# TobiaMarcucci/warm-start-hybrid-mpc

Measured on AMD Instinct MI355X. Metric: QP subproblems/sec, cart-pole-with-walls N=20 synthetic frontier, higher is better.
Workload: dtype f64

## Files before the change

### warm-start-hybrid-mpc_amd/csrc/hmpc_capi.hip

```cpp
#include <hip/hip_runtime.h>

#include <cmath>
#include <cstdio>
#include <cstdlib>
#include <cstring>
#include <memory>
#include <string>
#include <utility>
#include <vector>

#include "hmpc_device.h"

#include "hmpc_kernel.hip"
#include "hmpc_jit.h"
#include "hmpc_host.h"
#include "hmpc_shift.hip"
#include "hmpc_certify.hip"
#include "hmpc_branch.hip"
#include "hmpc_search.hip"

#define HMPC_CHECK_NODES 64

namespace {

struct StageHost {
    int m, mg;
    std::vector<double> C, h, scale;
    std::vector<int> rptr, rcol, cptr, crow, gptr, grow;
    std::vector<double> rval, cval, gval;
// ... 78 lines not shown
             "p.ring=%d;p.nd=%d;p.ndp=%d;p.ns=%d;p.nd_magic=%uu;p.nn_magic=%uu;p.split_lds=%d;p.static_rows=%d;p.polish_l1=%d;",
             p.nx, p.nu, p.nub, p.nuc, p.nz, p.T, p.nc, p.ncL, p.nT, p.mreg, p.Toff, p.M, p.Mpad, p.n, p.ne, p.nq, p.nr, p.nqT, p.n_primal, p.n_dual,
             p.mreg_magic, p.nnz0, p.nng0, p.reg.m, p.reg.mg, p.kcol, p.ngram, p.ring, p.nd, p.ndp, p.ns, p.nd_magic, p.nn_magic, p.split_lds,
             p.static_rows, p.polish_l1);
    return b;
}

static bool hmpc_sized_enabled()
{
    if (getenv("HMPC_FORCE_GENERIC") || getenv("HMPC_FORCE_BIG")) return false;
    if (const char *e = getenv("HMPC_JIT")) { if (atoi(e) == 0) return false; }
    if (const char *e = getenv("HMPC_JIT_SIZED")) { if (atoi(e) == 0) return false; }
    return true;
}

bool hmpc_jit_prepare_sized(const DevProb &p, hmpc_cfg (&cfg)[3], std::vector<void *> &libs, int &count_out, std::vector<std::string> *built)
{
    const std::string fields = hmpc_sized_fields(p);
    hmpc_jit_shape shapes[3];
    int slot[3], count = 0;
    int only = -1;
    if (const char *e = getenv("HMPC_WAVES")) { const int nw = atoi(e); only = nw == 1 || nw == 2 || nw == 4 ? hmpc_cfg_index(nw) : -1; }
    for (int c = 0; c < 3; c++) {
        const hmpc_kernel_choice &k = cfg[c].k;
        if (k.kc > 0) {
            int kf = 0, kb = 0, kt = 0;
            if (!hmpc_static_slots(p, k.waves, kf, kb, kt)) continue;
            if (kt < 1) kt = 1;
            shapes[count] = hmpc_jit_shape{p.nx, p.nu, p.nub, kf, kb, kt, k.waves, k.kc, fields};
            slot[count++] = c;
            continue;
        }
        if (k.big && c != (only >= 0 ? only : 2)) continue;
        int rs = p.Mpad / (WAVE << c), rs_max = 16;
        if (const char *e = getenv("HMPC_JIT_SIZED_ROWS")) rs_max = atoi(e);
        if (rs > rs_max) rs = 0;
        shapes[count] = hmpc_jit_shape{k.big ? -1 : 0, -1, 0, rs, 0, 0, 1 << c, 0, fields};
        slot[count++] = c;
    }
    if (!getenv("HMPC_JIT_SCHED")) {
        const uint64_t hsh = hmpc_jit::source_hash();
        for (int i = 0; i < count; i++) {
            hmpc_jit_shape probe = shapes[i];
            probe.ilp = 1;
// ... 53 lines not shown
{
    static const bool once = [] {
        if (getenv("HMPC_BACKTRACE")) { signal(SIGSEGV, hmpc_fatal_signal); signal(SIGABRT, hmpc_fatal_signal); signal(SIGBUS, hmpc_fatal_signal); }
        return true;
    }();
    (void)once;
}

namespace {

struct HostProblem {
    DevProb p{};
    StageHost reg;
    std::vector<double> ccv, Ct, ht, sct, P, PT, Cdn, sval;
    std::vector<int> cci, ei, ej, drow, rinfo, sptr, srow, nrow;
};

void split_rows(HostProblem &hp)
{
    DevProb &p = hp.p;
    const int nz = p.nz;
    const std::vector<double> &C = hp.reg.C;
    std::vector<int> &drow = hp.drow, &rinfo = hp.rinfo, &sptr = hp.sptr, &srow = hp.srow, &nrow = hp.nrow;
    std::vector<double> &sval = hp.sval, &Cdn = hp.Cdn;
    rinfo.assign(p.mreg, 0);
    sptr.assign(nz + 1, 0);
    sval.assign(p.mreg, 0.0);
    for (int r = 0; r < p.mreg; r++) {
        int cnt = 0, col = 0;
        for (int j = 0; j < nz; j++)
// ... 48 lines not shown
    p.dbg = getenv("HMPC_DBG") ? atoi(getenv("HMPC_DBG")) : 0;
    p.polish = opt ? opt->polish : 1;
    p.ptol = opt && opt->polish_tol > 0 ? opt->polish_tol : 1e-4;

    build_stage(q, q.F, q.G, q.h, q.nc, reg);
    p.reg.m = reg.m;
    p.reg.mg = reg.mg;
    p.mreg_magic = (unsigned)((0x100000000ULL + p.mreg - 1) / p.mreg);
    p.nnz0 = (int)reg.rcol.size();
    hp.ccv.assign((size_t)nz * HMPC_KC_STRIDE, 0.0);
    hp.cci.assign((size_t)nz * HMPC_KC_STRIDE, 0);
    p.kcol = 0;
    for (int j = 0; j < nz; j++) {
        const int len = reg.cptr[j + 1] - reg.cptr[j];
        if (len > p.kcol) p.kcol = len;
        for (int k = 0; k < len && k < HMPC_KC_STRIDE; k++) {
            hp.ccv[(size_t)j * HMPC_KC_STRIDE + k] = reg.cval[reg.cptr[j] + k];
            hp.cci[(size_t)j * HMPC_KC_STRIDE + k] = reg.crow[reg.cptr[j] + k];
        }
    }
    p.static_rows = (p.kcol <= HMPC_KC_STRIDE && p.mreg <= 255) ? 1 : 0;
    for (int r = 0; r < q.nc; r++) {
        int cnt = 0;
        for (int j = 0; j < nu; j++) cnt += reg.C[(size_t)r * nz + nx + j] != 0.0;
        if (cnt > 2) p.static_rows = 0;
    }
    p.nng0 = (int)reg.grow.size();
    for (int r = 0; r < q.nc; r++) {
        bool same = q.h_Tm1[r] == q.h[r];
        for (int j = 0; j < nx && same; j++) same = q.F_Tm1[r * nx + j] == q.F[r * nx + j];
// ... 38 lines not shown
        }
    p.cs = big > 0 ? 1.0 / big : 1.0;
    for (auto &v : P) v *= p.cs;
    for (auto &v : PT) v *= p.cs;
    {
        double cmin = 1.0;
        for (int i = 0; i < nz; i++) if (P[(size_t)i * nz + i] > 0) cmin = std::fmin(cmin, P[(size_t)i * nz + i]);
        for (int i = 0; i < nx; i++) if (PT[(size_t)i * nx + i] > 0) cmin = std::fmin(cmin, PT[(size_t)i * nx + i]);
        p.polish_l1 = cmin >= 1e-2 ? 1 : 0;
    }

    {
        std::vector<int> ei, ej;
        for (int i = 0; i < nz; i++)
            for (int j = 0; j <= i; j++) { ei.push_back(i); ej.push_back(j); }
        std::vector<int> order;
        for (int pass = 0; pass < 2; pass++)
            for (int e = 0; e < p.ne; e++)
                if ((reg.gptr[e + 1] > reg.gptr[e]) == (pass == 0)) order.push_back(e);
        p.ngram = 0;
        for (int e = 0; e < p.ne; e++) p.ngram += reg.gptr[e + 1] > reg.gptr[e];
        std::vector<int> gptr2(1, 0), grow2;
        std::vector<double> gval2;
        for (int e : order) {
            hp.ei.push_back(ei[e]); hp.ej.push_back(ej[e]);
            for (int k = reg.gptr[e]; k < reg.gptr[e + 1]; k++) { grow2.push_back(reg.grow[k]); gval2.push_back(reg.gval[k]); }
            gptr2.push_back((int)grow2.size());
        }
        reg.gptr.swap(gptr2); reg.grow.swap(grow2); reg.gval.swap(gval2);
        if (p.ngram > 128) p.static_rows = 0;
    }
    split_rows(hp);
    if (p.M >= 65536 || p.mreg >= 65536) return fail(HMPC_ETOOBIG, "more than 65535 constraint rows per node");
    return HMPC_OK;
}

int choose_kernels(DevProb &p, int lds_max, hmpc_cfg (&cfg)[3], std::vector<void *> &libs, int &jit_kernels, std::vector<std::string> *built)
{
    p.split_lds = 0;
    p.ring = 1;
    if (p.nz >= 16) {
        const bool big = hmpc_lds_bytes(p, 0, 0) > LDS_PER_CU || getenv("HMPC_FORCE_BIG");
        p.split_lds = 1;
        if (hmpc_lds_bytes(p, 0, big ? 1 : 0) > LDS_PER_CU) p.split_lds = 0;
    }
    for (int r = 2; r >= 1; r--) {
        p.ring = r;
        if (hmpc_lds_bytes(p, 0, 1) <= LDS_PER_CU) break;
    }
    if (const char *e = getenv("HMPC_RING")) {
        const int r = atoi(e);
        if (r >= 1 && r <= 2) p.ring = r;
// ... 3 lines not shown
        const bool sized = pass == 0 && hmpc_sized_enabled();
        if (pass == 0 && !sized) continue;
        for (int c = 0; c < 3; c++) { jit[c] = hmpc_kernel_choice{}; cfg[c] = hmpc_cfg{}; }
        jit_kernels = 0;
        if (sized) hmpc_jit_register_shapes(p, jit, LDS_PER_CU);
        for (int c = 0; c < 3; c++) {
            hmpc_cfg &cf = cfg[c];
            cf.k = hmpc_pick_kernel(p, 1 << c, jit);
            cf.lds = hmpc_lds_bytes(p, cf.k.kc, cf.k.big);
            if (cf.lds > LDS_PER_CU || (lds_max > 0 && cf.lds > (size_t)lds_max)) {
                char msg[256];
                snprintf(msg, sizeof msg, "problem needs %zu bytes of LDS per node, more than one CU has (%d)", cf.lds, lds_max > 0 ? lds_max : (int)LDS_PER_CU);
                return fail(HMPC_ETOOBIG, msg);
            }
        }
        if (!sized || hmpc_jit_prepare_sized(p, cfg, libs, jit_kernels, built)) break;
    }
    return HMPC_OK;
}

int resident_grid(size_t lds, int cus, const char *per_cu_env)
{
    int per_cu = (int)(LDS_PER_CU / lds);
    if (per_cu > 8) per_cu = 8;
    if (per_cu_env && atoi(per_cu_env) > 0) per_cu = atoi(per_cu_env);
    return (cus > 0 ? cus : 256) * per_cu;
}

struct CheckLayout {
    size_t obj, dobj, status, iters, idx, primal, dual, x0, fix, mirror, total;
};
// ... 129 lines not shown
    hmpc_install_backtrace();
    g_err.clear();
    if (!q || !out) return fail(HMPC_EINVAL, "null problem or output pointer");
    HostProblem hp;
    int rc = build_host_problem(*q, opt, hp);
    if (rc) return rc;
    int dev = opt ? opt->device : -1;
    if (dev < 0 && hipGetDevice(&dev) != hipSuccess) return fail(HMPC_EDEVICE, "no HIP device available");
    if (hipSetDevice(dev) != hipSuccess) return fail(HMPC_EDEVICE, "hipSetDevice failed");
    std::unique_ptr<hmpc_handle> h(new hmpc_handle());
    h->device = dev;
    h->dp = hp.p;
    int cus = 0, lds_max = 0;
    (void)hipDeviceGetAttribute(&cus, hipDeviceAttributeMultiprocessorCount, dev);
    (void)hipDeviceGetAttribute(&lds_max, hipDeviceAttributeMaxSharedMemoryPerBlock, dev);
    if ((rc = choose_kernels(h->dp, lds_max, h->cfg, h->jit_libs, h->jit_kernels, nullptr))) return rc;
    if ((rc = setup_device(h.get(), hp, *q, cus, lds_max))) return rc;
    if ((rc = hmpc_certify_setup(h.get(), cus))) return rc;
    *out = h.release();
    return HMPC_OK;
}

extern "C" int hmpc_jit_build_problem(const hmpc_problem *q, const hmpc_options *opt, char *paths, int32_t paths_len)
{
    g_err.clear();
    if (!q) return fail(HMPC_EINVAL, "null problem or output pointer");
    HostProblem hp;
    int rc = build_host_problem(*q, opt, hp);
    if (rc) return rc;
    hmpc_cfg cfg[3];
    std::vector<void *> libs;
    std::vector<std::string> built;
    int jit_kernels = 0;
    if ((rc = choose_kernels(hp.p, 0, cfg, libs, jit_kernels, &built))) return rc;
    if (paths && paths_len > 0) {
        std::string all;
        for (const std::string &b : built) all += b + "\n";
        snprintf(paths, (size_t)paths_len, "%s", all.c_str());
    }
    return HMPC_OK;
}

extern "C" int hmpc_destroy(hmpc_handle *h)
{
    if (!h) return HMPC_OK;
    (void)hipSetDevice(h->device);
    (void)hipDeviceSynchronize();
    delete h;
    return HMPC_OK;
// ... 355 lines not shown
```

### warm-start-hybrid-mpc_amd/csrc/hmpc_jit.h

```cpp
#ifndef HMPC_JIT_H
#define HMPC_JIT_H

#include <dlfcn.h>
#include <spawn.h>
#include <sys/stat.h>
#include <sys/wait.h>
#include <unistd.h>

#include <atomic>
#include <cerrno>
#include <climits>
#include <cstdint>
#include <cstdio>
#include <cstdlib>
#include <cstring>
#include <fstream>
#include <sstream>
#include <string>
#include <vector>

extern char **environ;

struct hmpc_jit_shape {
    int nx, nu, nub, kf, kb, kt, nw, kc;
    std::string sized;
    int ilp = 0;
};

namespace hmpc_jit {

inline std::string dir_of_library()
{
    Dl_info info;
    static int anchor;
    if (!dladdr((void *)&anchor, &info) || !info.dli_fname) return ".";
    std::string p = info.dli_fname;
    const size_t s = p.rfind('/');
    return s == std::string::npos ? "." : p.substr(0, s);
}

inline bool exists(const std::string &p) { struct stat st; return stat(p.c_str(), &st) == 0; }
// ... 103 lines not shown

inline uint64_t fnv(const std::string &t)
{
    uint64_t hsh = 1469598103934665603ull;
    for (char ch : t) { hsh ^= (unsigned char)ch; hsh *= 1099511628211ull; }
    return hsh;
}

inline std::string name_of(const hmpc_jit_shape &s, uint64_t hsh0)
{
    char b[160];
    const std::string fl = sched_flags(s) + "|" + safe_flags();
    const uint64_t hsh = hsh0 ^ fnv(fl);
    if (!s.sized.empty() && s.nx > 0) {
        snprintf(b, sizeof b, "hmpc_s_reg_%d_%d_%d_%d_%d_%d_w%d_kc%d%s_%016llx_%016llx", s.nx, s.nu, s.nub, s.kf, s.kb, s.kt, s.nw, s.kc, "",
                 (unsigned long long)fnv(s.sized), (unsigned long long)hsh);
        return b;
    }
    if (!s.sized.empty()) {
        snprintf(b, sizeof b, "hmpc_s_%s_w%d_r%d_%016llx_%016llx", s.nx < 0 ? "stream" : "generic", s.nw, s.kf, (unsigned long long)fnv(s.sized), (unsigned long long)hsh);
        return b;
    }
    return std::string();
}

inline std::vector<std::string> scrubbed_environment()
{
    static const char *const drop[] = {"LD_PRELOAD=", "ROCP", "ROCPROFILER", "ROCTRACER", "ROCTX", "HSA_TOOLS_LIB=", "HSA_TOOLS_REPORT_LOAD_FAILURE=", "HIP_TOOLS_LIB="};
    std::vector<std::string> env;
    for (char **e = environ; e && *e; e++) {
        bool keep = true;
// ... 24 lines not shown
    return tag;
}
inline unsigned next_build_seq() { static std::atomic<unsigned> n{0}; return n.fetch_add(1); }

inline pid_t start_build(const hmpc_jit_shape &s, const std::string &cache, uint64_t hsh, std::string &err, unsigned seq)
{
    const std::string base = cache + "/" + name_of(s, hsh), so = base + ".so";
    if (exists(so)) return 0;
    if (!exists(source_dir() + "/hmpc_kernel.hip")) { err = "kernel sources not found in " + source_dir(); return -1; }
    if (access(compiler().c_str(), X_OK) != 0) { err = "no compiler at " + compiler(); return -1; }
    const std::string tag = build_tag(seq);
    const std::string src = base + tag + ".hip", tmp = base + tag + ".tmp.so";
    {
        std::ofstream out(src);
        out << "// generated by hmpc_jit.h\n#define HMPC_KERNEL_ONLY\n#define hmpc_qp_kernel hmpc_qp_kernel_jit\n";
        if (s.nx > 0) out << "#define HMPC_JIT_KC " << s.kc << "\n";
        if (!s.sized.empty()) out << "#define HMPC_SIZED(p) " << s.sized << "\n";
        std::stringstream args;
        if (s.nx > 0) args << s.nx << ", " << s.nu << ", " << s.nub << ", " << s.kf << ", " << s.kb << ", " << s.kt << ", " << s.nw;
        else args << s.nx << ", -1, 0, " << s.kf << ", 0, 0, " << s.nw;
        out << "#include \"hmpc_device.h\"\n#include \"hmpc_kernel.hip\"\nHMPC_INSTANCE(" << args.str() << ")\nextern \"C\" void hmpc_jit_kernels(void **cold, void **warm)\n{\n    *cold = (void *)hmpc_qp_kernel<"
            << args.str() << ", false>;\n    *warm = (void *)hmpc_qp_kernel<" << args.str() << ", true>;\n}\nextern \"C\" const char *hmpc_jit_sized(void) { return \"" << s.sized << "\"; }\n";
        if (!out) { err = "cannot write " + src; return -1; }
    }
    const std::string cmd = compiler() + " --offload-arch=" + arch() + " -O3 -fPIC -std=c++17 -ffp-contract=fast -Wno-pass-failed " + quoted_flags(s) + " -I '" + include_dir() + "' -I '" +
                            source_dir() + "' -shared -Wl,-Bsymbolic -o '" + tmp + "' '" + src + "' > '" + base + tag + ".log' 2>&1 && mv '" + tmp + "' '" + so + "'";
    pid_t pid = -1;
    const char *argv[] = {"sh", "-c", cmd.c_str(), nullptr};
    const std::vector<std::string> env = scrubbed_environment();
    std::vector<char *> envp;
    for (const std::string &e : env) envp.push_back(const_cast<char *>(e.c_str()));
// ... 62 lines not shown
```

### warm-start-hybrid-mpc_amd/csrc/hmpc_kernel.hip

```cpp
#include <hip/hip_runtime.h>
#include <math.h>
#include <stdint.h>
#include <type_traits>

#include "hmpc_device.h"

#define WAVE 64
#define HMPC_REFINE_FROM_IT 12
#define HMPC_POLISH_RHO 1e5
#define HMPC_POLISH_RHO2 1e7
#define HMPC_POLISH_DELTA 1e-10
#define HMPC_RHO_OF(level) ((level) == 1 ? HMPC_POLISH_RHO2 : HMPC_POLISH_RHO)
#define HMPC_POLISH_ITERS 5
#define HMPC_POLISH_ROUNDS 6
#define HMPC_POLISH_ROUNDS_LAST 10
#define HMPC_ESC_MAX 2
#define HMPC_ESC_ITERS 6
#define HMPC_ESC_ENABLED(D) true
#define HMPC_LAM0_ROW 1
#ifndef HMPC_STABLE_DEN
#define HMPC_STABLE_DEN 1
#endif
#ifndef HMPC_PAIR
#define HMPC_PAIR 1
// ... 322 lines not shown
                a1 += c1 * v1;
                a2 += c2 * v2;
                a3 += c3 * v3;
            }
            for (; j < nz; j++) a0 += c[j] * v[j];
            return (a0 + a1) + (a2 + a3);
        }
    }
    if (lr < p.mreg) return row_dot(stage_lists<D>(S), lr, v);
    const int nz = D::nz(p);
    const double *c = p.Ct + (size_t)(lr - p.mreg) * nz;
    double a = 0;
    for (int j = 0; j < nz; j++) a += c[j] * v[j];
    return a;
}
template <class D> DEV double ccol_dot(const DevProb &p, const Lds &S, int t, int j, const ldsd *base)
{
    double a;
    if constexpr (D::kKC > 0) {
        const ldsd *eb = base + t * p.mreg, *cv = S.ccv + j * D::kKC;
        const ldsb *ci = S.cci + j * D::kKC;
        constexpr int H = D::kKC / 2;
        static_assert(D::kKC % 2 == 0, "padded columns come in two halves");
        double a0 = 0, a1 = 0;
#pragma unroll
        for (int hb = 0; hb < D::kKC; hb += H) {
            int idx[H];
            double cc[H], ee[H];
#pragma unroll
            for (int q = 0; q < H; q++) idx[q] = ci[hb + q];
#pragma unroll
            for (int q = 0; q < H; q++) cc[q] = cv[hb + q];
            HMPC_FENCE();
#pragma unroll
            for (int q = 0; q < H; q++) { HMPC_CHK(idx[q] >= 0 && idx[q] < p.mreg && j >= 0 && j < D::nz(p) && t >= 0 && t < p.T, 1); ee[q] = eb[idx[q]]; }
            HMPC_FENCE();
#pragma unroll
            for (int q = 0; q < H; q++) {
                if (q & 1) a1 += cc[q] * ee[q];
                else a0 += cc[q] * ee[q];
            }
        }
        a = a0 + a1;
    } else if (D::kBig && S.Cdn) {
        const int nz = D::nz(p);
        const ldsd *eb = base + t * p.mreg, *c = S.Cdn + j;
        double a0 = 0, a1 = 0;
        int r = 0;
        for (; r + 2 <= p.nd; r += 2) {
            a0 += c[r * nz] * eb[S.drow[r]];
            a1 += c[(r + 1) * nz] * eb[S.drow[r + 1]];
        }
        if (r < p.nd) a0 += c[r * nz] * eb[S.drow[r]];
// ... 807 lines not shown
{
    constexpr int NX = D::kNX, NU = D::kNU, NUB = D::kNUB, NUC = NU - NUB, NZ = NX + NU, NE = NZ * (NZ + 1) / 2;
    static_assert(NZ <= 16, "the register recursions broadcast inside one row of 16 lanes");
    constexpr int NXS = NX * (NX + 1) / 2, LMS = LM_STAGE(NX, NU), KG = D::kKC, GH = KG / 2;
    const int T = p.T;
    FSTAMP_DECL;
    LANE_OPAQUE(lane);
    if (lane == 0) S.flag[0] = 0;
    if (D::kNW == 1 || lane < WAVE) {
        const int ng = p.ngram;
        const bool has = lane < ng;
        const int ge = has ? lane : 0;
        const int gi = S.ei[ge], gj = S.ej[ge];
        const int gp0 = S.L0.gptr[ge], glen = has ? S.L0.gptr[ge + 1] - gp0 : 0;
        const double pij = S.P[gi * NZ + gj];
        ldsd *TG = S.Mm + NZ * NZ;
        for (int q = ng + lane; q < NE; q += WAVE) {
            const int i = S.ei[q], j = S.ej[q];
            const double a = S.P[i * NZ + j];
            S.Mm[i * NZ + j] = a;
            S.Mm[j * NZ + i] = a;
        }
        if (S.term_on) {
            const ldsd *Dt = S.e + p.Toff;
            if (p.nT == 0) {
                for (int q = lane; q < NZ * NZ; q += WAVE) TG[q] = 0.0;
            }
            for (int r0 = 0; r0 < p.nT; r0 += WAVE) {
                const int row = r0 + lane;
                const bool ok = row < p.nT;
// ... 23 lines not shown
#pragma unroll
        for (int i = 0; i < NX; i++) pn[i] = lane < NX ? S.PT[i * NX + lane] : 0.0;
        if (lane < NX) {
#pragma unroll
            for (int i = 0; i < NX; i++)
                if (i >= lane) S.Pr[T * NXS + sym(i, lane)] = pn[i];
        }
        int bad = 0;
        for (int t = T - 1; t >= 0; t--) {
            const ldsi *fx = S.fix + t * NUB;
            ldsd *Lm = S.Lm + t * LMS;
            int fxv[NUB];
#pragma unroll
            for (int b = 0; b < NUB; b++) fxv[b] = fx[b];
            double g0 = pij, g1 = 0.0;
            {
                const ldsd *Dt = S.e + t * p.mreg;
#pragma unroll
                for (int hb = 0; hb < KG; hb += GH) {
                    int idx[GH];
                    double gv[GH], dv[GH];
#pragma unroll
                    for (int q = 0; q < GH; q++) {
                        const int qq = gp0 + (hb + q < glen ? hb + q : 0);
                        idx[q] = S.L0.grow[qq];
                        gv[q] = S.L0.gval[qq];
                    }
                    HMPC_FENCE();
#pragma unroll
                    for (int q = 0; q < GH; q++) { HMPC_CHK(idx[q] >= 0 && idx[q] < p.mreg, 2); dv[q] = Dt[idx[q]]; }
                    HMPC_FENCE();
#pragma unroll
                    for (int q = 0; q < GH; q++) {
                        const double term = hb + q < glen ? gv[q] * dv[q] : 0.0;
                        if (q & 1) g1 += term;
                        else g0 += term;
                    }
                }
            }
            if (has) {
                S.Mm[gi * NZ + gj] = g0 + g1;
                S.Mm[gj * NZ + gi] = g0 + g1;
            }
            if (ng > WAVE) {
                const bool has2 = WAVE + lane < ng;
                const int ge2 = has2 ? WAVE + lane : 0;
                const int gi2 = S.ei[ge2], gj2 = S.ej[ge2];
                const int gq0 = S.L0.gptr[ge2], glen2 = has2 ? S.L0.gptr[ge2 + 1] - gq0 : 0;
                const ldsd *Dt = S.e + t * p.mreg;
                double h0 = S.P[gi2 * NZ + gj2], h1 = 0.0;
#pragma unroll
                for (int q = 0; q < KG; q++) {
                    const int qq = gq0 + (q < glen2 ? q : 0);
                    const double term = q < glen2 ? S.L0.gval[qq] * Dt[S.L0.grow[qq]] : 0.0;
// ... 650 lines not shown
    }
    __syncthreads();
    FSTAMP(10);
}

template <class D, int RS, class RM>
DEV void kkt_solve_reg(const DevProb &p, const Lds &S, Rows<RS> &R, const RM &rm, int lane, const ldsd *gsrc, double gs, bool usex0,
                       const ldsd *csrc, double cs, bool useb, ldsd *dw, ldsd *dlam, ldsd *dnuf FSTAMP_ARGS)
{
    constexpr int NX = D::kNX, NU = D::kNU, NUB = D::kNUB, NUC = NU - NUB, NZ = NX + NU;
    constexpr int NXS = NX * (NX + 1) / 2, LMS = LM_STAGE(NX, NU);
    const int T = p.T;
    FSTAMP_DECL;
    LANE_OPAQUE(lane);
    term_cols<D, RM>(p, S, lane, S.e);
    for (int o = lane; o < T * NZ; o += D::kNT) {
        const int t = o / NZ, j = o - t * NZ;
        const double a = (gsrc ? gs * gsrc[o] : 0.0) + ccol_dot<D>(p, S, t, j, S.e);
        S.g[o] = (useb ? S.g[o] : 0.0) - a;
    }
    for (int o = lane; o < T * NX; o += D::kNT) {
        const int t = o / NX, i = o - t * NX;
        double a = 0.0;
        if (csrc) {
#pragma unroll
            for (int l = 0; l < NX; l++) a += S.Pr[(t + 1) * NXS + sym(i, l)] * (cs * csrc[t * NX + l]);
        }
        S.pv[o] = a;
    }
    double pvr = 0.0;
    if (lane < NX) {
        pvr = -(gsrc ? gs * gsrc[T * NZ + lane] : 0.0);
        S.pv[T * NX + lane] = pvr;
    }
    __syncthreads();
// ... 150 lines not shown
                }
            }
        }
    }
    __syncthreads();
    const bool own_g = gsrc && gsrc != S.g;
    term_cols<D, RM>(p, S, lane, S.e);
    for (int o = lane; o < T * NUB; o += D::kNT) {
        const int t = o / NUB, b = o - t * NUB;
        double a = 0;
        if (S.fix[o] >= 0) {
            const int c = NX + NUC + b;
            a = own_g ? gs * gsrc[t * NZ + c] : 0.0;
#pragma unroll
            for (int j = 0; j < NZ; j++) a -= S.P[c * NZ + j] * dw[t * NZ + j];
            a -= ccol_dot<D>(p, S, t, c, S.e);
#pragma unroll
            for (int l = 0; l < NX; l++) a += S.AB[l * NZ + c] * dlam[(t + 1) * NX + l];
        }
        dnuf[o] = a;
    }
    if constexpr (HMPC_LAM0_ROW) {
        if (lane < NX) {
            double a = own_g ? gs * gsrc[lane] : 0.0;
#pragma unroll
            for (int j = 0; j < NZ; j++) a -= S.P[lane * NZ + j] * dw[j];
            a -= ccol_dot<D>(p, S, 0, lane, S.e);
#pragma unroll
            for (int l = 0; l < NX; l++) a += S.AB[l * NZ + lane] * dlam[NX + l];
            dlam[lane] = a;
        }
    }
    __syncthreads();
    FSTAMP(10);
}

template <class D, int RS, class RM>
DEV double kkt_solve_reg_pair(const DevProb &p, const Lds &S, Rows<RS> &R, const RM &rm, int lane, double tau FSTAMP_ARGS)
{
    constexpr int NX = D::kNX, NU = D::kNU, NUB = D::kNUB, NUC = NU - NUB, NZ = NX + NU;
    constexpr int NXS = NX * (NX + 1) / 2, LMS = LM_STAGE(NX, NU);
    const int T = p.T;
    const int nslot = RS;
    ldsd *pv2 = S.edyn;
    FSTAMP_DECL;
    LANE_OPAQUE(lane);
    ROWS_BEGIN(k, rw)
        S.e[rw.e] = R.D(k, rw.e) * rm.h(p, S, k, rw);
    ROWS_END
    __syncthreads();
    term_cols<D, RM>(p, S, lane, S.e);
    for (int o = lane; o < T * NZ; o += D::kNT) {
        const int t = o / NZ, j = o - t * NZ;
        S.g[o] = S.g[o] - ccol_dot<D>(p, S, t, j, S.e);
    }
    for (int o = lane; o < (T + 1) * NX; o += D::kNT) S.pv[o] = 0.0;
    __syncthreads();
    ROWS_BEGIN(k, rw)
        double v = 0;
        const double d = R.D(k, rw.e);
        if (d != 0.0) {
            const double sr = R.s(k, rw.e), zr = d * sr;
            const double rc = sr - rm.h(p, S, k, rw) * tau + rm.dot(p, S, k, rw, S.w);
            const double dsr = sr * zr;
            v = dsr * frcp(sr) - 1.0 * (d * rc);
        }
        S.e[rw.e] = v;
        R.dz(k, rw.e) = v;
    ROWS_END
    __syncthreads();
    term_cols<D, RM>(p, S, lane, S.e);
    for (int o = lane; o < T * NZ; o += D::kNT) {
        const int t = o / NZ, j = o - t * NZ;
        const double a = -1.0 * S.rd[o] + ccol_dot<D>(p, S, t, j, S.e);
        S.w2[o] = 0.0 - a;
    }
    for (int o = lane; o < T * NX; o += D::kNT) {
        const int t = o / NX, i = o - t * NX;
        double a = 0.0;
#pragma unroll
        for (int l = 0; l < NX; l++) a += S.Pr[(t + 1) * NXS + sym(i, l)] * (-1.0 * S.rdyn[t * NX + l]);
        pv2[o] = a;
    }
    double pvrA = 0.0, pvrB = 0.0;
    if (lane < NX) {
        pvrB = -(-1.0 * S.rd[T * NZ + lane]);
        pv2[T * NX + lane] = pvrB;
    }
    __syncthreads();
    FSTAMP(6);
    LANE_OPAQUE(lane);
// ... 147 lines not shown
        if (d != 0.0) {
            z1 = d * rm.dot(p, S, k, rw, S.w1) - d * rm.h(p, S, k, rw);
            q2 += z1 * z1 * frcp(d);
        }
        S.e[rw.e] = z1;
    ROWS_END
    __syncthreads();
    term_cols<D, RM>(p, S, lane, S.e);
    for (int o = lane; o < T * NUB; o += D::kNT) {
        const int t = o / NUB, b = o - t * NUB;
        double a = 0;
        if (S.fix[o] >= 0) {
            const int c = NX + NUC + b;
#pragma unroll
            for (int j = 0; j < NZ; j++) a -= S.P[c * NZ + j] * S.w1[t * NZ + j];
            a -= ccol_dot<D>(p, S, t, c, S.e);
#pragma unroll
            for (int l = 0; l < NX; l++) a += S.AB[l * NZ + c] * S.lam1[(t + 1) * NX + l];
        }
        S.nuf1[o] = a;
    }
    if (lane < NX) {
        double a = 0.0;
#pragma unroll
        for (int j = 0; j < NZ; j++) a -= S.P[lane * NZ + j] * S.w1[j];
        a -= ccol_dot<D>(p, S, 0, lane, S.e);
#pragma unroll
        for (int l = 0; l < NX; l++) a += S.AB[l * NZ + lane] * S.lam1[NX + l];
        S.lam1[lane] = a;
    }
    __syncthreads();
    ROWS_BEGIN(k, rw)
        const double d = R.D(k, rw.e);
        double z2 = 0.0;
        if (d != 0.0) z2 = d * rm.dot(p, S, k, rw, S.w2) - R.dz(k, rw.e);
        S.e[rw.e] = z2;
    ROWS_END
    __syncthreads();
    term_cols<D, RM>(p, S, lane, S.e);
    for (int o = lane; o < T * NUB; o += D::kNT) {
        const int t = o / NUB, b = o - t * NUB;
        double a = 0;
        if (S.fix[o] >= 0) {
            const int c = NX + NUC + b;
            a = -1.0 * S.rd[t * NZ + c];
#pragma unroll
            for (int j = 0; j < NZ; j++) a -= S.P[c * NZ + j] * S.w2[t * NZ + j];
            a -= ccol_dot<D>(p, S, t, c, S.e);
#pragma unroll
            for (int l = 0; l < NX; l++) a += S.AB[l * NZ + c] * S.lam2[(t + 1) * NX + l];
        }
        S.nuf2[o] = a;
    }
    if (lane < NX) {
        double a = -1.0 * S.rd[lane];
#pragma unroll
        for (int j = 0; j < NZ; j++) a -= S.P[lane * NZ + j] * S.w2[j];
        a -= ccol_dot<D>(p, S, 0, lane, S.e);
#pragma unroll
        for (int l = 0; l < NX; l++) a += S.AB[l * NZ + lane] * S.lam2[NX + l];
        S.lam2[lane] = a;
    }
    __syncthreads();
    FSTAMP(10);
    return q2;
}

template <class D, int RS, class RM>
DEV void kkt_dispatch(const DevProb &p, const Lds &S, Rows<RS> &R, const RM &rm, int lane, const ldsd *gsrc, double gs, bool usex0,
                      const ldsd *csrc, double cs, bool useb, ldsd *dw, ldsd *dlam, ldsd *dnuf FSTAMP_ARGS)
{
    if constexpr (D::kNX > 0) kkt_solve_reg<D, RS>(p, S, R, rm, lane, gsrc, gs, usex0, csrc, cs, useb, dw, dlam, dnuf FSTAMP_PASS);
    else kkt_solve<D, RS>(p, S, R, rm, lane, gsrc, gs, usex0, csrc, cs, useb, dw, dlam, dnuf FSTAMP_PASS);
// ... 165 lines not shown
            S.e[rw.e] = R.z(k, rw.e);
        ROWS_END
        __syncthreads();
        wPw = 0;
        for (int o = lane; o < n; o += D::kNT) {
            const int t = o / nz < T ? o / nz : T;
            const int i = o - t * nz, dim = t < T ? nz : nx;
            const ldsd *PP = t < T ? S.P : S.PT;
            double a = 0;
            for (int j = 0; j < dim; j++) a += PP[i * dim + j] * S.w[t * nz + j];
            wPw += a * S.w[o];
        }
        double rdinf = 0, certinf = 0, fy = 0, yinf = 0;
        winf = 0;
        term_cols<D, RM>(p, S, lane, S.e);
        for (int o = lane; o < n; o += D::kNT) {
            const int t = o / nz < T ? o / nz : T;
            const int j = o - t * nz;
            double a = 0;
            if (t == T) {
                a = S.lam[T * nx + j];
            } else {
                if (j < nx) a += S.lam[t * nx + j];
                for (int l = 0; l < nx; l++) a -= S.AB[l * AB_STRIDE + j] * S.lam[(t + 1) * nx + l];
                if (j >= nx + nuc && S.fix[t * nub + (j - nx - nuc)] >= 0) a += S.nuf[t * nub + (j - nx - nuc)];
                a += ccol_dot<D>(p, S, t, j, S.e);
            }
            double pw = 0;
            {
                const int dim = t < T ? nz : nx;
                const ldsd *PP = t < T ? S.P : S.PT;
                for (int l = 0; l < dim; l++) pw += PP[j * dim + l] * S.w[t * nz + l];
            }
            const double v = pw + a;
            S.rd[o] = v;
            rdinf = fmax(rdinf, fabs(v));
            certinf = fmax(certinf, fabs(a));
            winf = fmax(winf, fabs(S.w[o]));
        }
        double rcinf = 0;
        for (int o = lane; o < T * nx; o += D::kNT) {
            const int t = o / nx, i = o - t * nx;
            double a = S.w[(t + 1) * nz + i];
            for (int l = 0; l < nz; l++) a -= S.AB[i * AB_STRIDE + l] * S.w[t * nz + l];
            S.rdyn[o] = a;
            rcinf = fmax(rcinf, fabs(a));
        }
        double hz = 0, sz = 0;
        zinf = 0;
        ROWS_BEGIN(k, rw)
            double a = 0;
            if (rm.active(p, S, k, rw)) {
                const double zr = R.z(k, rw.e), sr = R.s(k, rw.e), hh = rm.h(p, S, k, rw);
                a = sr - hh * tau + rm.dot(p, S, k, rw, S.w);
// ... 1038 lines not shown
```

Before: 656,200.

## Specialize column and Gram dot products to actual per-column lengths in JIT kernels

After: 598,700. -8.8%, worse.

```diff
diff --git a/warm-start-hybrid-mpc_amd/csrc/hmpc_capi.hip b/warm-start-hybrid-mpc_amd/csrc/hmpc_capi.hip
--- a/warm-start-hybrid-mpc_amd/csrc/hmpc_capi.hip
+++ b/warm-start-hybrid-mpc_amd/csrc/hmpc_capi.hip
@@ -13,6 +13,7 @@
 
 #include "hmpc_kernel.hip"
 #include "hmpc_jit.h"
+#include "hmpc_lists.h"
 #include "hmpc_host.h"
 #include "hmpc_shift.hip"
 #include "hmpc_certify.hip"
@@ -121,7 +122,7 @@
     return true;
 }
 
-bool hmpc_jit_prepare_sized(const DevProb &p, hmpc_cfg (&cfg)[3], std::vector<void *> &libs, int &count_out, std::vector<std::string> *built)
+bool hmpc_jit_prepare_sized(const DevProb &p, const std::vector<int> &collen, const hmpc_gram_lanes &gram, hmpc_cfg (&cfg)[3], std::vector<void *> &libs, int &count_out, std::vector<std::string> *built)
 {
     const std::string fields = hmpc_sized_fields(p);
     hmpc_jit_shape shapes[3];
@@ -135,6 +136,9 @@
             if (!hmpc_static_slots(p, k.waves, kf, kb, kt)) continue;
             if (kt < 1) kt = 1;
             shapes[count] = hmpc_jit_shape{p.nx, p.nu, p.nub, kf, kb, kt, k.waves, k.kc, fields};
+            if ((int)collen.size() == p.nz && p.nz <= 16)
+                shapes[count].cols = hmpc_col_class_defines(hmpc_build_col_classes(collen.data(), p.nx, p.nu, p.nub, p.T, k.waves, k.kc), p.T) +
+                                     (k.kc == std::max(2, (p.kcol + 1) / 2 * 2) ? hmpc_gram_lane_defines(gram) : std::string());
             slot[count++] = c;
             continue;
         }
@@ -218,6 +222,8 @@
     StageHost reg;
     std::vector<double> ccv, Ct, ht, sct, P, PT, Cdn, sval;
     std::vector<int> cci, ei, ej, drow, rinfo, sptr, srow, nrow;
+    std::vector<int> collen;
+    hmpc_gram_lanes gram;
 };
 
 void split_rows(HostProblem &hp)
@@ -296,6 +302,7 @@
     for (int j = 0; j < nz; j++) {
         const int len = reg.cptr[j + 1] - reg.cptr[j];
         if (len > p.kcol) p.kcol = len;
+        hp.collen.push_back(len);
         for (int k = 0; k < len && k < HMPC_KC_STRIDE; k++) {
             hp.ccv[(size_t)j * HMPC_KC_STRIDE + k] = reg.cval[reg.cptr[j] + k];
             hp.cci[(size_t)j * HMPC_KC_STRIDE + k] = reg.crow[reg.cptr[j] + k];
@@ -364,10 +371,16 @@
         std::vector<int> ei, ej;
         for (int i = 0; i < nz; i++)
             for (int j = 0; j <= i; j++) { ei.push_back(i); ej.push_back(j); }
-        std::vector<int> order;
-        for (int pass = 0; pass < 2; pass++)
-            for (int e = 0; e < p.ne; e++)
-                if ((reg.gptr[e + 1] > reg.gptr[e]) == (pass == 0)) order.push_back(e);
+        std::vector<int> order, glen(p.ne);
+        for (int e = 0; e < p.ne; e++) glen[e] = reg.gptr[e + 1] - reg.gptr[e];
+        if (p.ne <= 136) {
+            hp.gram = hmpc_build_gram_lanes(glen.data(), p.ne, std::max(2, (p.kcol + 1) / 2 * 2));
+            order.assign(hp.gram.order, hp.gram.order + p.ne);
+        } else {
+            for (int pass = 0; pass < 2; pass++)
+                for (int e = 0; e < p.ne; e++)
+                    if ((glen[e] > 0) == (pass == 0)) order.push_back(e);
+        }
         p.ngram = 0;
         for (int e = 0; e < p.ne; e++) p.ngram += reg.gptr[e + 1] > reg.gptr[e];
         std::vector<int> gptr2(1, 0), grow2;
@@ -385,7 +398,7 @@
     return HMPC_OK;
 }
 
-int choose_kernels(DevProb &p, int lds_max, hmpc_cfg (&cfg)[3], std::vector<void *> &libs, int &jit_kernels, std::vector<std::string> *built)
+int choose_kernels(DevProb &p, const std::vector<int> &collen, const hmpc_gram_lanes &gram, int lds_max, hmpc_cfg (&cfg)[3], std::vector<void *> &libs, int &jit_kernels, std::vector<std::string> *built)
 {
     p.split_lds = 0;
     p.ring = 1;
@@ -419,7 +432,7 @@
                 return fail(HMPC_ETOOBIG, msg);
             }
         }
-        if (!sized || hmpc_jit_prepare_sized(p, cfg, libs, jit_kernels, built)) break;
+        if (!sized || hmpc_jit_prepare_sized(p, collen, gram, cfg, libs, jit_kernels, built)) break;
     }
     return HMPC_OK;
 }
@@ -579,7 +592,7 @@
     int cus = 0, lds_max = 0;
     (void)hipDeviceGetAttribute(&cus, hipDeviceAttributeMultiprocessorCount, dev);
     (void)hipDeviceGetAttribute(&lds_max, hipDeviceAttributeMaxSharedMemoryPerBlock, dev);
-    if ((rc = choose_kernels(h->dp, lds_max, h->cfg, h->jit_libs, h->jit_kernels, nullptr))) return rc;
+    if ((rc = choose_kernels(h->dp, hp.collen, hp.gram, lds_max, h->cfg, h->jit_libs, h->jit_kernels, nullptr))) return rc;
     if ((rc = setup_device(h.get(), hp, *q, cus, lds_max))) return rc;
     if ((rc = hmpc_certify_setup(h.get(), cus))) return rc;
     *out = h.release();
@@ -597,7 +610,7 @@
     std::vector<void *> libs;
     std::vector<std::string> built;
     int jit_kernels = 0;
-    if ((rc = choose_kernels(hp.p, 0, cfg, libs, jit_kernels, &built))) return rc;
+    if ((rc = choose_kernels(hp.p, hp.collen, hp.gram, 0, cfg, libs, jit_kernels, &built))) return rc;
     if (paths && paths_len > 0) {
         std::string all;
         for (const std::string &b : built) all += b + "\n";
diff --git a/warm-start-hybrid-mpc_amd/csrc/hmpc_jit.h b/warm-start-hybrid-mpc_amd/csrc/hmpc_jit.h
--- a/warm-start-hybrid-mpc_amd/csrc/hmpc_jit.h
+++ b/warm-start-hybrid-mpc_amd/csrc/hmpc_jit.h
@@ -25,6 +25,7 @@
     int nx, nu, nub, kf, kb, kt, nw, kc;
     std::string sized;
     int ilp = 0;
+    std::string cols;
 };
 
 namespace hmpc_jit {
@@ -158,7 +159,7 @@
     const uint64_t hsh = hsh0 ^ fnv(fl);
     if (!s.sized.empty() && s.nx > 0) {
         snprintf(b, sizeof b, "hmpc_s_reg_%d_%d_%d_%d_%d_%d_w%d_kc%d%s_%016llx_%016llx", s.nx, s.nu, s.nub, s.kf, s.kb, s.kt, s.nw, s.kc, "",
-                 (unsigned long long)fnv(s.sized), (unsigned long long)hsh);
+                 (unsigned long long)fnv(s.sized + s.cols), (unsigned long long)hsh);
         return b;
     }
     if (!s.sized.empty()) {
@@ -213,7 +214,7 @@
     {
         std::ofstream out(src);
         out << "// generated by hmpc_jit.h\n#define HMPC_KERNEL_ONLY\n#define hmpc_qp_kernel hmpc_qp_kernel_jit\n";
-        if (s.nx > 0) out << "#define HMPC_JIT_KC " << s.kc << "\n";
+        if (s.nx > 0) out << "#define HMPC_JIT_KC " << s.kc << "\n" << s.cols;
         if (!s.sized.empty()) out << "#define HMPC_SIZED(p) " << s.sized << "\n";
         std::stringstream args;
         if (s.nx > 0) args << s.nx << ", " << s.nu << ", " << s.nub << ", " << s.kf << ", " << s.kb << ", " << s.kt << ", " << s.nw;
diff --git a/warm-start-hybrid-mpc_amd/csrc/hmpc_kernel.hip b/warm-start-hybrid-mpc_amd/csrc/hmpc_kernel.hip
--- a/warm-start-hybrid-mpc_amd/csrc/hmpc_kernel.hip
+++ b/warm-start-hybrid-mpc_amd/csrc/hmpc_kernel.hip
@@ -360,29 +360,74 @@
     for (int j = 0; j < nz; j++) a += c[j] * v[j];
     return a;
 }
-template <class D> DEV double ccol_dot(const DevProb &p, const Lds &S, int t, int j, const ldsd *base)
+#ifndef HMPC_TIGHT_COLS
+#define HMPC_TIGHT_COLS 1
+#endif
+#if HMPC_TIGHT_COLS && defined(HMPC_SIZED) && defined(HMPC_JIT_COLCLS)
+#define HMPC_COLS_TIGHT 1
+struct ColCls {
+    static constexpr int cls[] = {HMPC_JIT_COLCLS};
+    static constexpr int N = sizeof(cls) / sizeof(int) / 2;
+    static constexpr unsigned long long perm = HMPC_JIT_COLPERM;
+    static constexpr int first(int c) { int k = 0; for (int i = 0; i < c; i++) k += cls[2 * i]; return k; }
+    static constexpr int trips(int c) { int k = 0; for (int i = 0; i < c; i++) k += (HMPC_JIT_T * cls[2 * i] + WAVE - 1) / WAVE; return k; }
+};
+template <class D, int C = 0, class F> DEV void tight_cols(const DevProb &p, int lane, F &&f)
+{
+    if constexpr (C < ColCls::N) {
+        constexpr int NC = ColCls::cls[2 * C], LEN = ColCls::cls[2 * C + 1], K0 = ColCls::first(C), W0 = ColCls::trips(C) % D::kNW;
+        const int T = p.T;
+        for (int o = ((lane >> 6) + D::kNW - W0) % D::kNW * WAVE + (lane & (WAVE - 1)); o < T * NC; o += D::kNT) {
+            const int t = o / NC, j = (int)((ColCls::perm >> (4 * (K0 + o - t * NC))) & 15ull);
+            f(t, j, std::integral_constant<int, LEN>());
+        }
+        tight_cols<D, C + 1>(p, lane, f);
+    }
+}
+#else
+#define HMPC_COLS_TIGHT 0
+#endif
+#if HMPC_TIGHT_COLS && defined(HMPC_SIZED) && defined(HMPC_JIT_BINLEN)
+template <class D> struct ColLen { static constexpr int bin = HMPC_JIT_BINLEN, x0 = HMPC_JIT_X0LEN; };
+#else
+template <class D> struct ColLen { static constexpr int bin = D::kKC, x0 = D::kKC; };
+#endif
+#ifndef HMPC_TIGHT_GRAM
+#define HMPC_TIGHT_GRAM 1
+#endif
+#if HMPC_TIGHT_GRAM && defined(HMPC_SIZED) && defined(HMPC_JIT_GRAM_LONG)
+#define HMPC_GRAM_TIGHT 1
+#else
+#define HMPC_GRAM_TIGHT 0
+#endif
+constexpr int gram_pos0(int s, int gh) { return s < (gh + 1) / 2 ? 2 * s : gh + 2 * (s - (gh + 1) / 2); }
+constexpr int gram_pos1(int s, int gh) { return s < gh / 2 ? 2 * s + 1 : gh + 2 * (s - gh / 2) + 1; }
+template <class D, int LEN = D::kKC> DEV double ccol_dot(const DevProb &p, const Lds &S, int t, int j, const ldsd *base)
 {
     double a;
     if constexpr (D::kKC > 0) {
+        static_assert(LEN <= D::kKC, "a class is no longer than the padded column");
         const ldsd *eb = base + t * p.mreg, *cv = S.ccv + j * D::kKC;
         const ldsb *ci = S.cci + j * D::kKC;
         constexpr int H = D::kKC / 2;
         static_assert(D::kKC % 2 == 0, "padded columns come in two halves");
         double a0 = 0, a1 = 0;
 #pragma unroll
-        for (int hb = 0; hb < D::kKC; hb += H) {
+        for (int hb = 0; hb < LEN; hb += H) {
+            const int nq = LEN - hb < H ? LEN - hb : H;
             int idx[H];
             double cc[H], ee[H];
 #pragma unroll
-            for (int q = 0; q < H; q++) idx[q] = ci[hb + q];
-#pragma unroll
-            for (int q = 0; q < H; q++) cc[q] = cv[hb + q];
+            for (int q = 0; q < H; q++) if (q < nq) idx[q] = ci[hb + q];
+#pragma unroll
+            for (int q = 0; q < H; q++) if (q < nq) cc[q] = cv[hb + q];
             HMPC_FENCE();
 #pragma unroll
-            for (int q = 0; q < H; q++) { HMPC_CHK(idx[q] >= 0 && idx[q] < p.mreg && j >= 0 && j < D::nz(p) && t >= 0 && t < p.T, 1); ee[q] = eb[idx[q]]; }
+            for (int q = 0; q < H; q++) if (q < nq) { HMPC_CHK(idx[q] >= 0 && idx[q] < p.mreg && j >= 0 && j < D::nz(p) && t >= 0 && t < p.T, 1); ee[q] = eb[idx[q]]; }
             HMPC_FENCE();
 #pragma unroll
             for (int q = 0; q < H; q++) {
+                if (q >= nq) continue;
                 if (q & 1) a1 += cc[q] * ee[q];
                 else a0 += cc[q] * ee[q];
             }
@@ -1220,6 +1265,14 @@
         const int gi = S.ei[ge], gj = S.ej[ge];
         const int gp0 = S.L0.gptr[ge], glen = has ? S.L0.gptr[ge + 1] - gp0 : 0;
         const double pij = S.P[gi * NZ + gj];
+#if HMPC_GRAM_TIGHT
+        constexpr int GNL = HMPC_JIT_GRAM_LONG, GNS = GNL > 0 ? (GH + 1) / 2 * 2 : GH;
+        const bool gpart = lane >= ng && lane < ng + GNL;
+        const int gkind = gpart ? 2 : lane < GNL ? 1 : 0;
+        const int te = gpart ? lane - ng : ge;
+        const int tp0 = S.L0.gptr[te], tlen = (has || gpart) ? S.L0.gptr[te + 1] - tp0 : 0;
+        const int gsrc = lane < GNL ? lane + ng : lane;
+#endif
         ldsd *TG = S.Mm + NZ * NZ;
         for (int q = ng + lane; q < NE; q += WAVE) {
             const int i = S.ei[q], j = S.ej[q];
@@ -1273,6 +1326,34 @@
 #pragma unroll
             for (int b = 0; b < NUB; b++) fxv[b] = fx[b];
             double g0 = pij, g1 = 0.0;
+#if HMPC_GRAM_TIGHT
+            {
+                const ldsd *Dt = S.e + t * p.mreg;
+                int idx[GNS];
+                double gv[GNS], dv[GNS];
+                bool ok[GNS];
+#pragma unroll
+                for (int s = 0; s < GNS; s++) {
+                    const int pos = gkind == 0 ? s : gkind == 1 ? gram_pos0(s, GH) : gram_pos1(s, GH);
+                    ok[s] = pos < tlen && (gkind != 0 || s < GH);
+                    const int qq = tp0 + (ok[s] ? pos : 0);
+                    idx[s] = S.L0.grow[qq];
+                    gv[s] = S.L0.gval[qq];
+                }
+                HMPC_FENCE();
+#pragma unroll
+                for (int s = 0; s < GNS; s++) { HMPC_CHK(idx[s] >= 0 && idx[s] < p.mreg, 2); dv[s] = Dt[idx[s]]; }
+                HMPC_FENCE();
+#pragma unroll
+                for (int s = 0; s < GNS; s++) {
+                    const double term = ok[s] ? gv[s] * dv[s] : 0.0;
+                    const bool to0 = gkind == 1 || (gkind == 0 && !(s & 1));
+                    g0 += to0 ? term : 0.0;
+                    g1 += to0 ? 0.0 : term;
+                }
+                g1 = __shfl(g1, gsrc);
+            }
+#else
             {
                 const ldsd *Dt = S.e + t * p.mreg;
 #pragma unroll
@@ -1297,6 +1378,7 @@
                     }
                 }
             }
+#endif
             if (has) {
                 S.Mm[gi * NZ + gj] = g0 + g1;
                 S.Mm[gj * NZ + gi] = g0 + g1;
@@ -1977,11 +2059,19 @@
     FSTAMP_DECL;
     LANE_OPAQUE(lane);
     term_cols<D, RM>(p, S, lane, S.e);
+#if HMPC_COLS_TIGHT
+    tight_cols<D>(p, lane, [&](int t, int j, auto len) {
+        const int o = t * NZ + j;
+        const double a = (gsrc ? gs * gsrc[o] : 0.0) + ccol_dot<D, decltype(len)::value>(p, S, t, j, S.e);
+        S.g[o] = (useb ? S.g[o] : 0.0) - a;
+    });
+#else
     for (int o = lane; o < T * NZ; o += D::kNT) {
         const int t = o / NZ, j = o - t * NZ;
         const double a = (gsrc ? gs * gsrc[o] : 0.0) + ccol_dot<D>(p, S, t, j, S.e);
         S.g[o] = (useb ? S.g[o] : 0.0) - a;
     }
+#endif
     for (int o = lane; o < T * NX; o += D::kNT) {
         const int t = o / NX, i = o - t * NX;
         double a = 0.0;
@@ -2162,7 +2252,7 @@
             a = own_g ? gs * gsrc[t * NZ + c] : 0.0;
 #pragma unroll
             for (int j = 0; j < NZ; j++) a -= S.P[c * NZ + j] * dw[t * NZ + j];
-            a -= ccol_dot<D>(p, S, t, c, S.e);
+            a -= ccol_dot<D, ColLen<D>::bin>(p, S, t, c, S.e);
 #pragma unroll
             for (int l = 0; l < NX; l++) a += S.AB[l * NZ + c] * dlam[(t + 1) * NX + l];
         }
@@ -2173,7 +2263,7 @@
             double a = own_g ? gs * gsrc[lane] : 0.0;
 #pragma unroll
             for (int j = 0; j < NZ; j++) a -= S.P[lane * NZ + j] * dw[j];
-            a -= ccol_dot<D>(p, S, 0, lane, S.e);
+            a -= ccol_dot<D, ColLen<D>::x0>(p, S, 0, lane, S.e);
 #pragma unroll
             for (int l = 0; l < NX; l++) a += S.AB[l * NZ + lane] * dlam[NX + l];
             dlam[lane] = a;
@@ -2198,10 +2288,17 @@
     ROWS_END
     __syncthreads();
     term_cols<D, RM>(p, S, lane, S.e);
+#if HMPC_COLS_TIGHT
+    tight_cols<D>(p, lane, [&](int t, int j, auto len) {
+        const int o = t * NZ + j;
+        S.g[o] = S.g[o] - ccol_dot<D, decltype(len)::value>(p, S, t, j, S.e);
+    });
+#else
     for (int o = lane; o < T * NZ; o += D::kNT) {
         const int t = o / NZ, j = o - t * NZ;
         S.g[o] = S.g[o] - ccol_dot<D>(p, S, t, j, S.e);
     }
+#endif
     for (int o = lane; o < (T + 1) * NX; o += D::kNT) S.pv[o] = 0.0;
     __syncthreads();
     ROWS_BEGIN(k, rw)
@@ -2218,11 +2315,19 @@
     ROWS_END
     __syncthreads();
     term_cols<D, RM>(p, S, lane, S.e);
+#if HMPC_COLS_TIGHT
+    tight_cols<D>(p, lane, [&](int t, int j, auto len) {
+        const int o = t * NZ + j;
+        const double a = -1.0 * S.rd[o] + ccol_dot<D, decltype(len)::value>(p, S, t, j, S.e);
+        S.w2[o] = 0.0 - a;
+    });
+#else
     for (int o = lane; o < T * NZ; o += D::kNT) {
         const int t = o / NZ, j = o - t * NZ;
         const double a = -1.0 * S.rd[o] + ccol_dot<D>(p, S, t, j, S.e);
         S.w2[o] = 0.0 - a;
     }
+#endif
     for (int o = lane; o < T * NX; o += D::kNT) {
         const int t = o / NX, i = o - t * NX;
         double a = 0.0;
@@ -2400,7 +2505,7 @@
             const int c = NX + NUC + b;
 #pragma unroll
             for (int j = 0; j < NZ; j++) a -= S.P[c * NZ + j] * S.w1[t * NZ + j];
-            a -= ccol_dot<D>(p, S, t, c, S.e);
+            a -= ccol_dot<D, ColLen<D>::bin>(p, S, t, c, S.e);
 #pragma unroll
             for (int l = 0; l < NX; l++) a += S.AB[l * NZ + c] * S.lam1[(t + 1) * NX + l];
         }
@@ -2410,7 +2515,7 @@
         double a = 0.0;
 #pragma unroll
         for (int j = 0; j < NZ; j++) a -= S.P[lane * NZ + j] * S.w1[j];
-        a -= ccol_dot<D>(p, S, 0, lane, S.e);
+        a -= ccol_dot<D, ColLen<D>::x0>(p, S, 0, lane, S.e);
 #pragma unroll
         for (int l = 0; l < NX; l++) a += S.AB[l * NZ + lane] * S.lam1[NX + l];
         S.lam1[lane] = a;
@@ -2432,7 +2537,7 @@
             a = -1.0 * S.rd[t * NZ + c];
 #pragma unroll
             for (int j = 0; j < NZ; j++) a -= S.P[c * NZ + j] * S.w2[t * NZ + j];
-            a -= ccol_dot<D>(p, S, t, c, S.e);
+            a -= ccol_dot<D, ColLen<D>::bin>(p, S, t, c, S.e);
 #pragma unroll
             for (int l = 0; l < NX; l++) a += S.AB[l * NZ + c] * S.lam2[(t + 1) * NX + l];
         }
@@ -2442,7 +2547,7 @@
         double a = -1.0 * S.rd[lane];
 #pragma unroll
         for (int j = 0; j < NZ; j++) a -= S.P[lane * NZ + j] * S.w2[j];
-        a -= ccol_dot<D>(p, S, 0, lane, S.e);
+        a -= ccol_dot<D, ColLen<D>::x0>(p, S, 0, lane, S.e);
 #pragma unroll
         for (int l = 0; l < NX; l++) a += S.AB[l * NZ + lane] * S.lam2[NX + l];
         S.lam2[lane] = a;
@@ -2638,6 +2743,30 @@
         double rdinf = 0, certinf = 0, fy = 0, yinf = 0;
         winf = 0;
         term_cols<D, RM>(p, S, lane, S.e);
+#if HMPC_COLS_TIGHT
+        auto rd_entry = [&](int o, int t, int j, double a) {
+            double pw = 0;
+            {
+                const int dim = t < T ? nz : nx;
+                const ldsd *PP = t < T ? S.P : S.PT;
+                for (int l = 0; l < dim; l++) pw += PP[j * dim + l] * S.w[t * nz + l];
+            }
+            const double v = pw + a;
+            S.rd[o] = v;
+            rdinf = fmax(rdinf, fabs(v));
+            certinf = fmax(certinf, fabs(a));
+            winf = fmax(winf, fabs(S.w[o]));
+        };
+        tight_cols<D>(p, lane, [&](int t, int j, auto len) {
+            double a = 0;
+            if (j < nx) a += S.lam[t * nx + j];
+            for (int l = 0; l < nx; l++) a -= S.AB[l * AB_STRIDE + j] * S.lam[(t + 1) * nx + l];
+            if (j >= nx + nuc && S.fix[t * nub + (j - nx - nuc)] >= 0) a += S.nuf[t * nub + (j - nx - nuc)];
+            a += ccol_dot<D, decltype(len)::value>(p, S, t, j, S.e);
+            rd_entry(t * nz + j, t, j, a);
+        });
+        for (int o = T * nz + lane; o < n; o += D::kNT) rd_entry(o, T, o - T * nz, S.lam[T * nx + (o - T * nz)]);
+#else
         for (int o = lane; o < n; o += D::kNT) {
             const int t = o / nz < T ? o / nz : T;
             const int j = o - t * nz;
@@ -2662,6 +2791,7 @@
             certinf = fmax(certinf, fabs(a));
             winf = fmax(winf, fabs(S.w[o]));
         }
+#endif
         double rcinf = 0;
         for (int o = lane; o < T * nx; o += D::kNT) {
             const int t = o / nx, i = o - t * nx;
diff --git a/warm-start-hybrid-mpc_amd/csrc/hmpc_lists.h b/warm-start-hybrid-mpc_amd/csrc/hmpc_lists.h
--- /dev/null
+++ b/warm-start-hybrid-mpc_amd/csrc/hmpc_lists.h
@@ -0,0 +1,170 @@
+#ifndef HMPC_LISTS_H
+#define HMPC_LISTS_H
+
+#include <cstdio>
+#include <string>
+
+#define HMPC_COL_CLASSES 3
+
+struct hmpc_col_classes {
+    int ncls = 0;
+    int count[HMPC_COL_CLASSES] = {};
+    int len[HMPC_COL_CLASSES] = {};
+    int perm[16] = {};
+    int binlen = 0;
+    int x0len = 0;
+    int slots = 0, slots_padded = 0;
+    bool tight = false;
+};
+
+inline int hmpc_col_slots(const int *count, const int *len, int ncls, int T, int nw)
+{
+    int per[4] = {0, 0, 0, 0}, w = 0;
+    for (int c = 0; c < ncls; c++)
+        for (int trip = 0; trip < (T * count[c] + 63) / 64; trip++, w++) per[w % nw] += len[c];
+    int m = 0;
+    for (int i = 0; i < nw; i++) m = per[i] > m ? per[i] : m;
+    return m;
+}
+
+inline hmpc_col_classes hmpc_build_col_classes(const int *collen, int nx, int nu, int nub, int T, int nw, int kc)
+{
+    hmpc_col_classes r;
+    const int nz = nx + nu;
+    if (nz < 1 || nz > 16 || nw < 1 || nw > 4) return r;
+    for (int j = 0; j < nz; j++) r.perm[j] = j;
+    for (int i = 1; i < nz; i++)
+        for (int k = i; k > 0 && collen[r.perm[k]] > collen[r.perm[k - 1]]; k--) { const int s = r.perm[k]; r.perm[k] = r.perm[k - 1]; r.perm[k - 1] = s; }
+    for (int j = 0; j < nx; j++) r.x0len = collen[j] > r.x0len ? collen[j] : r.x0len;
+    for (int j = nz - nub; j < nz; j++) r.binlen = collen[j] > r.binlen ? collen[j] : r.binlen;
+    r.slots_padded = (T * nz + 64 * nw - 1) / (64 * nw) * kc;
+    int best = -1;
+    for (int a = 1; a <= nz; a++)
+        for (int b = a; b <= nz; b++) {
+            int cnt[HMPC_COL_CLASSES], ln[HMPC_COL_CLASSES], n = 0;
+            const int lo[3] = {0, a, b}, hi[3] = {a, b, nz};
+            for (int c = 0; c < 3; c++)
+                if (hi[c] > lo[c]) { cnt[n] = hi[c] - lo[c]; ln[n] = collen[r.perm[lo[c]]]; n++; }
+            const int s = hmpc_col_slots(cnt, ln, n, T, nw);
+            if (best < 0 || s < best || (s == best && n < r.ncls)) {
+                best = s;
+                r.ncls = n;
+                for (int c = 0; c < n; c++) { r.count[c] = cnt[c]; r.len[c] = ln[c]; }
+            }
+        }
+    r.slots = best;
+    r.tight = best < r.slots_padded;
+    if (!r.tight) {
+        r.ncls = 1;
+        r.count[0] = nz;
+        r.len[0] = kc;
+        for (int j = 0; j < nz; j++) r.perm[j] = j;
+        r.slots = r.slots_padded;
+    }
+    return r;
+}
+
+inline std::string hmpc_col_class_defines(const hmpc_col_classes &c, int T)
+{
+    std::string s;
+    if (c.tight) {
+        s = "#define HMPC_JIT_T " + std::to_string(T) + "\n#define HMPC_JIT_COLCLS ";
+        for (int k = 0; k < c.ncls; k++) s += (k ? ", " : "") + std::to_string(c.count[k]) + ", " + std::to_string(c.len[k]);
+        unsigned long long perm = 0;
+        int nz = 0;
+        for (int k = 0; k < c.ncls; k++) nz += c.count[k];
+        for (int k = 0; k < nz; k++) perm |= (unsigned long long)c.perm[k] << (4 * k);
+        char b[32];
+        snprintf(b, sizeof b, "0x%llxull", perm);
+        s += std::string("\n#define HMPC_JIT_COLPERM ") + b + "\n";
+    }
+    s += "#define HMPC_JIT_BINLEN " + std::to_string(c.binlen) + "\n#define HMPC_JIT_X0LEN " + std::to_string(c.x0len) + "\n";
+    return s;
+}
+
+
+inline double hmpc_col_product(const double *cv, const int *ci, int kc, int len, const double *e)
+{
+    const int H = kc / 2;
+    double a0 = 0, a1 = 0;
+    for (int hb = 0; hb < kc; hb += H)
+        for (int q = 0; q < H && hb + q < len; q++) {
+            if (q & 1) a1 += cv[hb + q] * e[ci[hb + q]];
+            else a0 += cv[hb + q] * e[ci[hb + q]];
+        }
+    return a0 + a1;
+}
+
+struct hmpc_gram_lanes {
+    int ngram = 0, nlong = 0, slots = 0;
+    bool tight = false;
+    int order[136] = {};
+};
+
+inline int hmpc_gram_pos0(int s, int gh) { return s < (gh + 1) / 2 ? 2 * s : gh + 2 * (s - (gh + 1) / 2); }
+inline int hmpc_gram_pos1(int s, int gh) { return s < gh / 2 ? 2 * s + 1 : gh + 2 * (s - gh / 2) + 1; }
+
+inline hmpc_gram_lanes hmpc_build_gram_lanes(const int *glen, int ne, int kc)
+{
+    hmpc_gram_lanes r;
+    if (ne < 0 || ne > 136) return r;
+    const int gh = kc / 2;
+    int n = 0, longest = 0;
+    for (int e = 0; e < ne; e++)
+        if (glen[e] > 0) { r.order[n++] = e; longest = glen[e] > longest ? glen[e] : longest; }
+    r.ngram = n;
+    for (int i = 1; i < n; i++)
+        for (int k = i; k > 0 && glen[r.order[k]] > glen[r.order[k - 1]]; k--) { const int s = r.order[k]; r.order[k] = r.order[k - 1]; r.order[k - 1] = s; }
+    for (int e = 0; e < ne; e++)
+        if (glen[e] <= 0) r.order[n++] = e;
+    for (int i = 0; i < r.ngram; i++) r.nlong += glen[r.order[i]] > gh;
+    r.slots = r.nlong > 0 ? (gh + 1) / 2 * 2 : gh;
+    r.tight = kc >= 2 && longest <= kc && r.ngram >= 1 && r.ngram <= 64 && r.nlong <= 64 - r.ngram;
+    return r;
+}
+
+inline std::string hmpc_gram_lane_defines(const hmpc_gram_lanes &g)
+{
+    return g.tight ? "#define HMPC_JIT_GRAM_LONG " + std::to_string(g.nlong) + "\n" : std::string();
+}
+
+inline double hmpc_gram_padded(const double *val, const int *row, int len, int kc, const double *d, double pij)
+{
+    const int gh = kc / 2;
+    double g0 = pij, g1 = 0.0;
+    for (int hb = 0; hb < kc; hb += gh)
+        for (int q = 0; q < gh; q++) {
+            const double term = hb + q < len ? val[hb + q] * d[row[hb + q]] : 0.0;
+            if (q & 1) g1 += term;
+            else g0 += term;
+        }
+    return g0 + g1;
+}
+
+inline void hmpc_gram_lane(const double *val, const int *row, int len, int kc, int slots, int kind, const double *d, double pij, double &g0, double &g1, int *walked)
+{
+    const int gh = kc / 2;
+    g0 = pij;
+    g1 = 0.0;
+    for (int s = 0; s < slots; s++) {
+        const int pos = kind == 0 ? s : kind == 1 ? hmpc_gram_pos0(s, gh) : hmpc_gram_pos1(s, gh);
+        const bool ok = pos < len && (kind != 0 || s < gh);
+        const double term = ok ? val[pos] * d[row[pos]] : 0.0;
+        if (ok && walked) walked[pos]++;
+        const bool to0 = kind == 1 || (kind == 0 && !(s & 1));
+        g0 += to0 ? term : 0.0;
+        g1 += to0 ? 0.0 : term;
+    }
+}
+
+inline double hmpc_gram_tight(const double *val, const int *row, int len, int kc, int slots, const double *d, double pij, int *walked)
+{
+    const int gh = kc / 2;
+    double g0, g1, h0, h1;
+    if (len <= gh) { hmpc_gram_lane(val, row, len, kc, slots, 0, d, pij, g0, g1, walked); return g0 + g1; }
+    hmpc_gram_lane(val, row, len, kc, slots, 1, d, pij, g0, g1, walked);
+    hmpc_gram_lane(val, row, len, kc, slots, 2, d, 0.0, h0, h1, walked);
+    return g0 + h1;
+}
+
+#endif
```
